# ZrrSkywalker/MonoDETR

Measured on AMD Instinct MI355X. Metric: training images/sec at B=8 per GPU, KITTI 384x1280, higher is better.
Workload: dtype bf16; 1 GPU; full MonoDETR training step (ResNet-50 + depth predictor + 3 enc / 3 dec layers, 550 train queries, 4 levels, criterion + AdamW) = BASELINE configs[2] (1 GPU) / configs[3] (DDP); global_batch=8, per_gpu_batch=8, image=3x384x1280, queries=50, precision=bf16, parallelism=dp1, grad_sync=none, prime_steps=12, launch=one hipGraph replay per iteration, cpu_affinity=NUMA node 1 of the GPU

## Files before the change

include/monodetr_amd.h:

```cpp
#ifndef MONODETR_AMD_H
#define MONODETR_AMD_H

#include <stdint.h>

#ifdef __cplusplus
extern "C" {
#endif

#define MDETR_ABI_VERSION 17

#define MDETR_F32 0
#define MDETR_F64 1
#define MDETR_BF16 2

#define MDETR_OK            0
#define MDETR_E_ARG        -1
#define MDETR_E_HIP        -2
#define MDETR_E_ALIGN      -3
#define MDETR_E_UNSUPPORTED -4

int mdetr_abi_version(void);
const char *mdetr_last_error(void);

int mdetr_msda_forward(int dtype,
                       const void *value, const int64_t *spatial_shapes, const int64_t *level_start,
                       const void *loc, const void *attn, void *out,
                       int B, int S, int M, int D, int L, int Lq, int P,
                       int device, void *stream);

int mdetr_msda_backward(int dtype,
                        const void *value, const int64_t *spatial_shapes, const int64_t *level_start,
                        const void *loc, const void *attn, const void *grad_out,
                        void *grad_value, void *grad_loc, void *grad_attn,
                        int B, int S, int M, int D, int L, int Lq, int P,
                        int device, void *stream);

int mdetr_msda_forward_cpu(int dtype,
                           const void *value, const int64_t *spatial_shapes, const int64_t *level_start,
                           const void *loc, const void *attn, void *out,
                           int B, int S, int M, int D, int L, int Lq, int P);
int mdetr_msda_backward_cpu(int dtype,
                            const void *value, const int64_t *spatial_shapes, const int64_t *level_start,
// ... 93 lines not shown
                            float alpha, float fg_weight, float bg_weight, float depth_min, float depth_max,
                            const float *grad_out, float *grad_logits, int device, void *stream);

int mdetr_adamw_step(int param_dtype, void *param, float *master, const void *grad, float *exp_avg, float *exp_avg_sq,
                     int64_t n, int64_t n_no_decay, float beta1, float beta2, float eps, float weight_decay,
                     float step_size, const float *step_size_dev, int device, void *stream);
int mdetr_adamw_step_counted(int param_dtype, void *param, float *master, const void *grad, float *exp_avg, float *exp_avg_sq,
                             int64_t n, int64_t n_no_decay, float beta1, float beta2, float eps, float weight_decay,
                             const double *step_count_dev, float lr, const double *lr_dev, int device, void *stream);
int mdetr_adamw_step_gathered(int param_dtype, void *param, float *master, const void *const *grad_ptrs, int ntensors,
                              const int *tensor_block_begin, const int64_t *flat_offsets, const int64_t *nbytes, const int *block_tensor,
                              const int64_t *block_start, int chunk_bytes, float *exp_avg, float *exp_avg_sq, int64_t n_no_decay,
                              float beta1, float beta2, float eps, float weight_decay, float step_size, const float *step_size_dev,
                              const double *step_count_dev, float lr, const double *lr_dev, int device, void *stream);

#define MDETR_TGEMM_RELU 1
#define MDETR_TGEMM_NN 2
#define MDETR_TGEMM_BIAS_F32 4
#define MDETR_TGEMM_OUT_F32 8
int mdetr_tgemm(const void *a, const void *w, const void *bias, const void *res, void *y, int64_t T, int N, int K,
                int64_t lda, int64_t ldw, int64_t ldr, int64_t ldy, int flags, float dropout_p, uint64_t seed,
                const void *seed_dev, int device, void *stream);
int mdetr_tgemm_masked(const void *a, const void *w, const void *res, const void *mask, void *y, int64_t T, int N, int K,
                       int64_t lda, int64_t ldw, int64_t ldr, int64_t ldm, int64_t ldy, int device, void *stream);
int mdetr_tgemm_f32(const void *a, const void *w, const void *bias, const void *res, void *y, int64_t T, int N, int K,
                    int64_t lda, int64_t ldw, int64_t ldr, int64_t ldy, int flags, float dropout_p, uint64_t seed,
                    const void *seed_dev, int device, void *stream);
int mdetr_tgemm_f32_masked(const void *a, const void *w, const void *res, const void *mask, void *y, int64_t T, int N, int K,
                           int64_t lda, int64_t ldw, int64_t ldr, int64_t ldm, int64_t ldy, int device, void *stream);

#define MDETR_SGEMM_NT 0
#define MDETR_SGEMM_NN 1
#define MDETR_SGEMM_TN 2
#define MDETR_SGEMM_MAX_PROBLEMS 10
#define MDETR_SGEMM_MAX_TERMS 5
typedef struct {
    const void *a, *b;
    int64_t lda, ldb;
    int32_t k, a_dtype, b_dtype, pad_;
} mdetr_sgemm_term;
typedef struct {
    mdetr_sgemm_term term[MDETR_SGEMM_MAX_TERMS];
    void *c;
    const float *bias;
    float *colsum;
    const float *mask;
    const void *res;
    int64_t ldc, ldm, ldr;
    int32_t nterm, m, n, relu_cols, c_dtype, res_dtype;
} mdetr_sgemm_problem;
int64_t mdetr_sgemm_workspace_bytes(int mode, const mdetr_sgemm_problem *problems, int nprob);
int mdetr_sgemm_grouped(int mode, const mdetr_sgemm_problem *problems, int nprob, void *workspace, int64_t workspace_bytes, int device, void *stream);

#define MDETR_KITTI_FLIP 1u
#define MDETR_KITTI_DISTORT 2u
#define MDETR_KITTI_CONTRAST_FIRST 4u
#define MDETR_KITTI_BRIGHTNESS 8u
#define MDETR_KITTI_CONTRAST 16u
#define MDETR_KITTI_SATURATION 32u
#define MDETR_KITTI_HUE 64u
typedef struct MdetrKittiImage {
    int64_t pixel_offset;
    int32_t width, height;
    uint32_t flags;
    uint32_t perm;
    float brightness, contrast, saturation, hue;
// ... 134 lines not shown
```

monodetr_amd/_capi.py:

```python
import ctypes
import os
import threading

_HERE = os.path.dirname(os.path.abspath(__file__))
LIB_PATH = os.environ.get("MDETR_LIB_PATH") or os.path.join(_HERE, "libmonodetr_amd.so")

MDETR_F32, MDETR_F64, MDETR_BF16 = 0, 1, 2
MDETR_E_UNSUPPORTED = -4
ABI_VERSION = 17

_c_int, _c_vp = ctypes.c_int, ctypes.c_void_p

SIGNATURES = {
    "mdetr_abi_version": (_c_int, []),
    "mdetr_last_error": (ctypes.c_char_p, []),
    "mdetr_msda_variant": (_c_int, [_c_int] * 5),
    "mdetr_msda_forward": (_c_int, [_c_int] + [_c_vp] * 6 + [_c_int] * 7 + [_c_int, _c_vp]),
    "mdetr_msda_backward": (_c_int, [_c_int] + [_c_vp] * 9 + [_c_int] * 7 + [_c_int, _c_vp]),
    "mdetr_msda_forward_cpu": (_c_int, [_c_int] + [_c_vp] * 6 + [_c_int] * 7),
    "mdetr_msda_backward_cpu": (_c_int, [_c_int] + [_c_vp] * 9 + [_c_int] * 7),
    "mdetr_msda_backward_ex": (_c_int, [_c_int] + [_c_vp] * 9 + [_c_int] * 7 + [_c_vp, _c_vp, _c_vp, ctypes.c_int64] + [_c_int, _c_vp]),
    "mdetr_msda_backward_workspace_bytes": (ctypes.c_int64, [_c_int, _c_vp, _c_vp] + [_c_int] * 7),
    "mdetr_msda_indices": (_c_int, [_c_int] + [_c_vp] * 3 + [_c_int] * 5 + [_c_int, _c_vp]),
    "mdetr_attn_forward": (_c_int, [_c_int] + [_c_vp] * 6 + [_c_int] * 4 + [ctypes.c_int64] * 3 + [_c_int] * 3
                           + [ctypes.c_float, ctypes.c_float, ctypes.c_uint64, _c_vp, _c_int, _c_vp]),
    "mdetr_attn_backward": (_c_int, [_c_int] + [_c_vp] * 11 + [_c_int] * 4 + [ctypes.c_int64] * 3 + [_c_int] * 3
                            + [ctypes.c_float, ctypes.c_float, ctypes.c_uint64, _c_vp, _c_int, _c_vp]),
    "mdetr_lsa_forward": (_c_int, [_c_vp] * 3 + [_c_int] * 5 + [ctypes.c_int64] * 3 + [_c_int, _c_vp]),
    "mdetr_ddn_loss_forward": (_c_int, [_c_vp] * 4 + [_c_int] * 5 + [ctypes.c_int64] * 4 + [ctypes.c_float] * 5 + [_c_vp, _c_vp, _c_int, _c_vp]),
    "mdetr_ddn_loss_backward": (_c_int, [_c_vp] * 4 + [_c_int] * 5 + [ctypes.c_int64] * 4 + [ctypes.c_float] * 5 + [_c_vp, _c_vp, _c_int, _c_vp]),
    "mdetr_pair_losses_workspace_bytes": (ctypes.c_int64, [_c_int, _c_int]),
    "mdetr_pair_losses_forward": (_c_int, [_c_vp] * 14 + [_c_int] * 6 + [ctypes.c_float, ctypes.c_float] + [_c_vp] * 4 + [_c_int, _c_vp]),
    "mdetr_pair_losses_backward": (_c_int, [_c_vp] * 13 + [_c_int] * 6 + [ctypes.c_float, ctypes.c_float] + [_c_vp] * 8 + [_c_int, _c_vp]),
    "mdetr_adamw_step": (_c_int, [_c_int] + [_c_vp] * 5 + [ctypes.c_int64] * 2 + [ctypes.c_float] * 5 + [_c_vp, _c_int, _c_vp]),
    "mdetr_adamw_step_gathered": (_c_int, [_c_int, _c_vp, _c_vp, _c_vp, _c_int] + [_c_vp] * 5 + [_c_int, _c_vp, _c_vp, ctypes.c_int64] + [ctypes.c_float] * 5
                                  + [_c_vp, _c_vp, ctypes.c_float, _c_vp, _c_int, _c_vp]),
    "mdetr_adamw_step_counted": (_c_int, [_c_int] + [_c_vp] * 5 + [ctypes.c_int64] * 2 + [ctypes.c_float] * 4 + [_c_vp, ctypes.c_float, _c_vp, _c_int, _c_vp]),
    "mdetr_tgemm": (_c_int, [_c_vp] * 5 + [ctypes.c_int64, _c_int, _c_int] + [ctypes.c_int64] * 4 + [_c_int, ctypes.c_float, ctypes.c_uint64, _c_vp, _c_int, _c_vp]),
    "mdetr_sgemm_workspace_bytes": (ctypes.c_int64, [_c_int, _c_vp, _c_int]),
    "mdetr_sgemm_grouped": (_c_int, [_c_int, _c_vp, _c_int, _c_vp, ctypes.c_int64, _c_int, _c_vp]),
    "mdetr_tgemm_masked": (_c_int, [_c_vp] * 5 + [ctypes.c_int64, _c_int, _c_int] + [ctypes.c_int64] * 5 + [_c_int, _c_vp]),
    "mdetr_tgemm_f32": (_c_int, [_c_vp] * 5 + [ctypes.c_int64, _c_int, _c_int] + [ctypes.c_int64] * 4 + [_c_int, ctypes.c_float, ctypes.c_uint64, _c_vp, _c_int, _c_vp]),
# ... 119 lines not shown
```

monodetr_amd/csrc/sgemm.hip:

```cpp
#include <hip/hip_runtime.h>
#include <stdint.h>

#include <mdetr_wave.h>

#include "msda.h"
#include "sgemm.h"

namespace mdetr {
namespace {

constexpr int kTile = 64, kSlab = 32, kPitchK = kSlab + 4, kPitchN = kTile + 4, kTnTile = 64, kTnWaves = 4, kTnMaxSplit = 16;
constexpr int kMaxTerms = 24;
constexpr int kFlagCBf16 = 1, kFlagResBf16 = 2;

struct Term {
    const void *a, *b;
    int64_t lda, ldb;
    int K, a_bf16, b_bf16, pad_;
};
struct Prob {
    void *c;
    const float *bias;
    float *colsum;
    const float *mask;
    const void *res;
    int64_t ldc, ldm, ldr;
    int M, N, relu_cols, term0, nterm, tile0, tiles_n, flags;
    int foff, pad_;
};
struct Args {
    Term t[kMaxTerms];
    Prob p[MDETR_SGEMM_MAX_PROBLEMS];
    int nprob;
    int split, flat;
    float *ws;
};

// ... 451 lines not shown
            const float *slot = red + wave * 64 * 64;
#pragma unroll
            for (int q = 0; q < 4; ++q) {
#pragma unroll
                for (int r = 0; r < 16; ++r) acc[q >> 1][q & 1][r] += slot[(q * 16 + r) * 64 + lane];
            }
        }
    }
    if (wave != 0) return;
    float sum = 0.f;
#pragma unroll
    for (int w = 0; w < kTnWaves; ++w) sum += cred[w * 64 + lane];
    const int mm = tm * kTnTile + lane;
    if (split == 1) {
#pragma unroll
        for (int q = 0; q < 4; ++q)
            epilogue_tile(P, tm * kTnTile + (q >> 1), 2, tn * kTnTile + 2 * li + (q & 1), lh, acc[q >> 1][q & 1]);
        if (P.colsum && tn == 0 && mm < PM) as_global_rw<float>(P.colsum)[mm] = sum;
        return;
    }
    MDETR_GLOBAL float *part = as_global_rw<float>(largs.ws) + static_cast<int64_t>(blockIdx.y) * largs.flat + P.foff;
#pragma unroll
    for (int q = 0; q < 4; ++q) {
        const int col = tn * kTnTile + 2 * li + (q & 1);
#pragma unroll
        for (int r = 0; r < 16; ++r) {
            const int row = tm * kTnTile + (q >> 1) + 2 * ((r & 3) + 8 * (r >> 2) + 4 * lh);
            if (row < PM && col < PN) part[static_cast<int64_t>(row) * PN + col] = acc[q >> 1][q & 1][r];
        }
    }
    if (tn == 0 && mm < PM) part[static_cast<int64_t>(PM) * PN + mm] = sum;
}

__global__ __launch_bounds__(256)
void sgemm_tn_reduce(const Args a)
{
    __shared__ __attribute__((aligned(16))) Args largs;
    {
        const unsigned *src = reinterpret_cast<const unsigned *>(&a);
        unsigned *dst = reinterpret_cast<unsigned *>(&largs);
        for (unsigned i = threadIdx.x; i < sizeof(Args) / 4; i += blockDim.x) dst[i] = src[i];
        __syncthreads();
    }
    const int f = blockIdx.x * 256 + threadIdx.x, flat = largs.flat;
    if (f >= flat) return;
    int pi = 0;
    for (int i = 1; i < largs.nprob; ++i)
        if (f >= largs.p[i].foff) pi = i;
    const Prob &P = largs.p[pi];
    const MDETR_GLOBAL float *part = as_global<float>(largs.ws) + f;
    float v = 0.f;
    for (int s2 = 0; s2 < largs.split; ++s2) v += part[static_cast<int64_t>(s2) * flat];
    const int e = f - P.foff, mn = P.M * P.N;
    if (e < mn) {
        const int row = e / P.N, col = e - row * P.N;
        const int64_t o = static_cast<int64_t>(row) * P.ldc + col;
        if (P.flags & kFlagCBf16) as_global_rw<__bf16>(P.c)[o] = static_cast<__bf16>(v);
        else as_global_rw<float>(P.c)[o] = v;
    } else if (P.colsum) {
        as_global_rw<float>(P.colsum)[e - mn] = v;
    }
}

int tn_split(const mdetr_sgemm_problem *p, int nprob)
{
    int tiles = 0, kmin = 1 << 30;
    for (int i = 0; i < nprob; ++i) {
        tiles += ((p[i].m + kTnTile - 1) / kTnTile) * ((p[i].n + kTnTile - 1) / kTnTile);
        kmin = p[i].term[0].k < kmin ? p[i].term[0].k : kmin;
    }
    int s = (768 + tiles - 1) / tiles;
    const int by_rows = kmin / (64 * kTnWaves);
    s = s < by_rows ? s : by_rows;
    return s < 1 ? 1 : (s > kTnMaxSplit ? kTnMaxSplit : s);
}

int64_t tn_flat(const mdetr_sgemm_problem *p, int nprob)
{
    int64_t f = 0;
    for (int i = 0; i < nprob; ++i) f += static_cast<int64_t>(p[i].m) * p[i].n + p[i].m;
    return f;
}

bool dtype_ok(int d) { return d == MDETR_F32 || d == MDETR_BF16; }

}

const char *sgemm_check(int mode, const mdetr_sgemm_problem *p, int nprob)
{
    if (mode != MDETR_SGEMM_NT && mode != MDETR_SGEMM_NN && mode != MDETR_SGEMM_TN) return "unknown mode";
    if (!p || nprob <= 0 || nprob > MDETR_SGEMM_MAX_PROBLEMS) return "1 .. MDETR_SGEMM_MAX_PROBLEMS problems per group";
    int terms = 0;
    for (int i = 0; i < nprob; ++i) {
        const mdetr_sgemm_problem &q = p[i];
        if (q.m <= 0 || q.n <= 0 || q.nterm <= 0 || q.nterm > MDETR_SGEMM_MAX_TERMS) return "bad shape (m, n > 0; 1 .. MDETR_SGEMM_MAX_TERMS terms)";
        if (!q.c || q.ldc < q.n || !dtype_ok(q.c_dtype)) return "bad result (null, row stride < n, or element type)";
        if (q.relu_cols < 0 || q.relu_cols > q.n) return "relu_cols outside [0, n]";
        if (q.mask && q.ldm < q.n) return "mask row stride < n";
        if (q.res && (q.ldr < q.n || !dtype_ok(q.res_dtype))) return "bad res (row stride < n, or element type)";
        if (mode == MDETR_SGEMM_TN && (q.nterm != 1 || q.bias || q.mask || q.res || q.relu_cols)) return "TN: one term, no bias / relu / mask / res";
        if (mode != MDETR_SGEMM_TN && q.colsum) return "colsum belongs to TN";
        for (int t = 0; t < q.nterm; ++t) {
            const mdetr_sgemm_term &x = q.term[t];
            if (!x.a || !x.b || x.k <= 0 || !dtype_ok(x.a_dtype) || !dtype_ok(x.b_dtype)) return "bad term (null operand, k <= 0, or element type)";
            const int64_t a_cols = mode == MDETR_SGEMM_TN ? q.m : x.k, b_cols = mode == MDETR_SGEMM_NT ? x.k : q.n;
            if (x.lda < a_cols || x.ldb < b_cols) return "operand row stride shorter than its row";
        }
        terms += q.nterm;
    }
    if (terms > kMaxTerms) return "too many terms in one group";
    if (mode == MDETR_SGEMM_TN && tn_flat(p, nprob) >= (1ll << 31)) return "TN group too large";
    return nullptr;
}

int64_t sgemm_workspace_bytes(int mode, const mdetr_sgemm_problem *p, int nprob)
{
    if (mode != MDETR_SGEMM_TN) return 0;
    const int split = tn_split(p, nprob);
    return split > 1 ? static_cast<int64_t>(split) * tn_flat(p, nprob) * 4 : 0;
}

hipError_t sgemm_launch(int mode, const mdetr_sgemm_problem *p, int nprob, void *workspace, hipStream_t st)
{
    Args a;
    a.split = 1; a.flat = 0; a.ws = nullptr;
    int tiles = 0, terms = 0;
    int64_t foff = 0;
    double flop = 0.0, bytes = 0.0;
    const int tsz = mode == MDETR_SGEMM_TN ? kTnTile : kTile;
    for (int i = 0; i < nprob; ++i) {
        const mdetr_sgemm_problem &q = p[i];
        Prob &P = a.p[i];
        P.c = q.c; P.bias = q.bias; P.colsum = q.colsum; P.mask = q.mask; P.res = q.res;
        P.ldc = q.ldc; P.ldm = q.ldm; P.ldr = q.ldr;
        P.M = q.m; P.N = q.n; P.relu_cols = q.relu_cols; P.term0 = terms; P.nterm = q.nterm;
        P.tile0 = tiles; P.tiles_n = (q.n + tsz - 1) / tsz;
        P.flags = (q.c_dtype == MDETR_BF16 ? kFlagCBf16 : 0) | (q.res && q.res_dtype == MDETR_BF16 ? kFlagResBf16 : 0);
        P.foff = static_cast<int>(foff); P.pad_ = 0;
        foff += static_cast<int64_t>(q.m) * q.n + q.m;
        tiles += ((q.m + tsz - 1) / tsz) * P.tiles_n;
        bytes += static_cast<double>(q.m) * q.n * (q.c_dtype == MDETR_BF16 ? 2.0 : 4.0) * (1.0 + (q.res ? 1.0 : 0.0)) + (q.mask ? 4.0 * q.m * q.n : 0.0);
        for (int t = 0; t < q.nterm; ++t) {
            const mdetr_sgemm_term &x = q.term[t];
            Term &T = a.t[terms++];
            T.a = x.a; T.b = x.b; T.lda = x.lda; T.ldb = x.ldb; T.K = x.k;
            T.a_bf16 = x.a_dtype == MDETR_BF16; T.b_bf16 = x.b_dtype == MDETR_BF16; T.pad_ = 0;
            flop += 2.0 * q.m * q.n * x.k;
            bytes += static_cast<double>(x.k) * (q.m * (T.a_bf16 ? 2.0 : 4.0) + q.n * (T.b_bf16 ? 2.0 : 4.0));
        }
    }
    a.nprob = nprob;
    ProfileScope prof(21, tiles, st, flop / 1e6, bytes / 1e3);
    if (mode == MDETR_SGEMM_TN) {
        a.split = tn_split(p, nprob);
        a.flat = static_cast<int>(tn_flat(p, nprob));
        a.ws = static_cast<float *>(workspace);
        hipLaunchKernelGGL(sgemm_tn_kernel, dim3(tiles, a.split), dim3(64 * kTnWaves), 0, st, a);
        if (a.split > 1) hipLaunchKernelGGL(sgemm_tn_reduce, dim3((a.flat + 255) / 256), dim3(256), 0, st, a);
    }
    else if (mode == MDETR_SGEMM_NN) hipLaunchKernelGGL(sgemm_kernel<true>, dim3(tiles), dim3(256), 0, st, a);
    else hipLaunchKernelGGL(sgemm_kernel<false>, dim3(tiles), dim3(256), 0, st, a);
    return hipGetLastError();
}

}
```

monodetr_amd/monodetr/heads.py:

```python
import os

import torch

from .. import sgemm_ext

ENABLED = os.environ.get("MDETR_HEADS") == "1"


def _heads_ok(x, bbox, dim, dep, ang, cls):
    from .depthaware_transformer import MLP
    if not ENABLED:
        return False
    if not (isinstance(bbox, MLP) and bbox.num_layers == 3 and all(isinstance(m, MLP) and m.num_layers == 2 for m in (dim, dep, ang))
            and isinstance(cls, torch.nn.Linear)):
        return False
    ps = [p for m in (bbox, dim, dep, ang, cls) for p in m.parameters()]
    if not all(p.dtype == torch.float32 and p.is_contiguous() for p in ps):
        return False
    C = x.shape[-1]
    firsts = [bbox.layers[0], dim.layers[0], dep.layers[0], ang.layers[0]]
    hid = firsts[0].out_features
    if not (all(l.in_features == C and l.out_features == hid and l.bias is not None for l in firsts) and cls.in_features == C
            and cls.bias is not None and bbox.layers[1].in_features == hid and bbox.layers[1].out_features == hid
            and all(m.layers[-1].bias is not None for m in (bbox, dim, dep, ang)) and bbox.layers[1].bias is not None):
        return False
    return x.dim() == 3 and x.is_contiguous() and sgemm_ext.usable(x.view(-1, C), *ps) and not torch.is_autocast_enabled()


class _HeadsLevel(torch.autograd.Function):

    @staticmethod
    def forward(ctx, x, w1b, b1b, w2b, b2b, w3b, b3b, w1d, b1d, wd, bd, w1p, b1p, wp, bp, w1a, b1a, wa, ba, wc, bc):
        ctx.set_materialize_grads(False)
        B, Q, C = x.shape
        T, hid = B * Q, w1b.shape[0]
        x2 = x.view(T, C)
        new = lambda n: torch.empty((T, n), dtype=torch.float32, device=x.device)
        h1, h2 = new(4 * hid), new(hid)
        delta, size, depth, angle, logits = new(w3b.shape[0]), new(wd.shape[0]), new(wp.shape[0]), new(wa.shape[0]), new(wc.shape[0])
        P, G = sgemm_ext.Problem, sgemm_ext.grouped
        sl = [slice(i * hid, (i + 1) * hid) for i in range(4)]
        G(sgemm_ext.NT, [P([(x2, w)], h1[:, s], bias=b, relu_cols=True) for w, b, s in zip((w1b, w1d, w1p, w1a), (b1b, b1d, b1p, b1a), sl)]
          + [P([(x2, wc)], logits, bias=bc)])
        G(sgemm_ext.NT, [P([(h1[:, sl[0]], w2b)], h2, bias=b2b, relu_cols=True), P([(h1[:, sl[1]], wd)], size, bias=bd),
                         P([(h1[:, sl[2]], wp)], depth, bias=bp), P([(h1[:, sl[3]], wa)], angle, bias=ba)])
        G(sgemm_ext.NT, [P([(h2, w3b)], delta, bias=b3b)])
        ctx.save_for_backward(x, h1, h2, w1b, w2b, w3b, w1d, wd, w1p, wp, w1a, wa, wc)
        shape = lambda t: t.view(B, Q, -1)
        return shape(delta), shape(size), shape(depth), shape(angle), shape(logits), x.view_as(x)

    @staticmethod
    @torch.autograd.function.once_differentiable
    def backward(ctx, g_delta, g_size, g_depth, g_angle, g_logits, g_skip):
        x, h1, h2, w1b, w2b, w3b, w1d, wd, w1p, wp, w1a, wa, wc = ctx.saved_tensors
        B, Q, C = x.shape
        T, hid = B * Q, w1b.shape[0]
        x2 = x.view(T, C)

        def flat(g, n):
            if g is None:
                return torch.zeros((T, n), dtype=torch.float32, device=x.device)
            return g.reshape(T, n).to(torch.float32).contiguous()
        g_delta, g_size, g_depth, g_angle, g_logits = (flat(g, w.shape[0]) for g, w in
                                                       ((g_delta, w3b), (g_size, wd), (g_depth, wp), (g_angle, wa), (g_logits, wc)))
        P, G = sgemm_ext.Problem, sgemm_ext.grouped
        sl = [slice(i * hid, (i + 1) * hid) for i in range(4)]
        new = lambda *s: torch.empty(s, dtype=torch.float32, device=x.device)
        dh2, dh1 = new(T, hid), new(T, 4 * hid)
        G(sgemm_ext.NN, [P([(g_delta, w3b)], dh2, mask=h2)])
        G(sgemm_ext.NN, [P([(g, w)], dh1[:, s], mask=h1[:, s]) for g, w, s in zip((dh2, g_size, g_depth, g_angle), (w2b, wd, wp, wa), sl)])
        dx = None
        if ctx.needs_input_grad[0]:
            dx = torch.empty_like(x)
            skip = g_skip.reshape(T, C) if g_skip is not None else None
            if skip is not None and not (skip.stride(1) == 1 and skip.dtype in (torch.float32, torch.bfloat16)):
                skip = skip.contiguous()
            G(sgemm_ext.NN, [P([(dh1[:, s], w) for s, w in zip(sl, (w1b, w1d, w1p, w1a))] + [(g_logits, wc)], dx.view(T, C), res=skip)])
        outs = {}
        jobs = []
        for key, dy, act, w in (("3b", g_delta, h2, w3b), ("2b", dh2, h1[:, sl[0]], w2b), ("d", g_size, h1[:, sl[1]], wd),
                                ("p", g_depth, h1[:, sl[2]], wp), ("a", g_angle, h1[:, sl[3]], wa),
                                ("1b", dh1[:, sl[0]], x2, w1b), ("1d", dh1[:, sl[1]], x2, w1d), ("1p", dh1[:, sl[2]], x2, w1p),
                                ("1a", dh1[:, sl[3]], x2, w1a), ("c", g_logits, x2, wc)):
            dw, db = torch.empty_like(w), new(w.shape[0])
            outs[key] = (dw, db)
            jobs.append(P([(dy, act)], dw, colsum=db))
        G(sgemm_ext.TN, jobs)
        o = outs
        return (dx, o["1b"][0], o["1b"][1], o["2b"][0], o["2b"][1], o["3b"][0], o["3b"][1], o["1d"][0], o["1d"][1], o["d"][0], o["d"][1],
                o["1p"][0], o["1p"][1], o["p"][0], o["p"][1], o["1a"][0], o["1a"][1], o["a"][0], o["a"][1], o["c"][0], o["c"][1])


def heads_level(x, bbox, dim, dep, ang, cls):
    if not _heads_ok(x, bbox, dim, dep, ang, cls):
        return None
    lb, ld, lp, la = bbox.layers, dim.layers, dep.layers, ang.layers
    return _HeadsLevel.apply(x, lb[0].weight, lb[0].bias, lb[1].weight, lb[1].bias, lb[2].weight, lb[2].bias,
                             ld[0].weight, ld[0].bias, ld[1].weight, ld[1].bias, lp[0].weight, lp[0].bias, lp[1].weight, lp[1].bias,
                             la[0].weight, la[0].bias, la[1].weight, la[1].bias, cls.weight, cls.bias)
```

monodetr_amd/sgemm_ext.py:

```python
import ctypes

import torch

from . import _capi

_backend = None
NT, NN, TN = 0, 1, 2
MAX_PROBLEMS, MAX_TERMS = 10, 5


class _Term(ctypes.Structure):
    _fields_ = [("a", ctypes.c_void_p), ("b", ctypes.c_void_p), ("lda", ctypes.c_int64), ("ldb", ctypes.c_int64),
                ("k", ctypes.c_int32), ("a_dtype", ctypes.c_int32), ("b_dtype", ctypes.c_int32), ("pad_", ctypes.c_int32)]


class _Problem(ctypes.Structure):
    _fields_ = [("term", _Term * MAX_TERMS), ("c", ctypes.c_void_p), ("bias", ctypes.c_void_p), ("colsum", ctypes.c_void_p),
                ("mask", ctypes.c_void_p), ("res", ctypes.c_void_p), ("ldc", ctypes.c_int64), ("ldm", ctypes.c_int64),
                ("ldr", ctypes.c_int64), ("nterm", ctypes.c_int32), ("m", ctypes.c_int32), ("n", ctypes.c_int32),
                ("relu_cols", ctypes.c_int32), ("c_dtype", ctypes.c_int32), ("res_dtype", ctypes.c_int32)]


def _lib():
    return _backend if _backend is not None else _capi.lib()


def _code(t):
    if t.dtype == torch.float32:
        return _capi.MDETR_F32
    if t.dtype == torch.bfloat16:
        return _capi.MDETR_BF16
    raise TypeError("sgemm: fp32 or bf16 operands, got %s" % t.dtype)


def _mat(t, what):
    if not (t.dim() == 2 and t.stride(1) == 1 and t.stride(0) >= t.shape[1]):
        raise ValueError("sgemm: %s must be 2-D with unit column stride, got shape %s strides %s" % (what, tuple(t.shape), t.stride()))
    return t


def usable(*tensors):
    for t in tensors:
        if t is None:
            continue
        if not ((t.is_cuda or _backend is not None) and t.dtype in (torch.float32, torch.bfloat16) and t.dim() in (1, 2) and t.stride(-1) == 1):
            return False
    return True


class Problem:

    def __init__(self, terms, out, bias=None, relu_cols=0, mask=None, res=None, colsum=None):
        self.terms, self.out, self.bias, self.mask, self.res, self.colsum = list(terms), out, bias, mask, res, colsum
        self.relu_cols = out.shape[1] if relu_cols is True else int(relu_cols)


def grouped(mode, problems):
    if not 0 < len(problems) <= MAX_PROBLEMS:
        raise ValueError("sgemm: 1 .. %d problems per group" % MAX_PROBLEMS)
    arr = (_Problem * len(problems))()
    dev = problems[0].out.device
    for q, pr in zip(arr, problems):
        out = _mat(pr.out, "out")
        M, N = out.shape
        if len(pr.terms) > MAX_TERMS:
            raise ValueError("sgemm: at most %d terms per problem" % MAX_TERMS)
        for i, (A, B) in enumerate(pr.terms):
            A, B = _mat(A, "A"), _mat(B, "B")
            if mode == NT:
                K = A.shape[1]
                ok = A.shape == (M, K) and B.shape == (N, K)
            elif mode == NN:
                K = A.shape[1]
                ok = A.shape == (M, K) and B.shape == (K, N)
            else:
                K = A.shape[0]
                ok = A.shape == (K, M) and B.shape == (K, N)
            if not ok:
                raise ValueError("sgemm: term %d shapes A %s B %s do not give [%d, %d] in mode %d" % (i, tuple(A.shape), tuple(B.shape), M, N, mode))
            t = q.term[i]
            t.a, t.b, t.lda, t.ldb, t.k, t.a_dtype, t.b_dtype = A.data_ptr(), B.data_ptr(), A.stride(0), B.stride(0), K, _code(A), _code(B)
        q.nterm, q.m, q.n, q.relu_cols = len(pr.terms), M, N, pr.relu_cols
        q.c, q.ldc, q.c_dtype = out.data_ptr(), out.stride(0), _code(out)
        if pr.bias is not None:
            assert pr.bias.dtype == torch.float32 and pr.bias.shape == (N,) and pr.bias.is_contiguous()
            q.bias = pr.bias.data_ptr()
        if pr.mask is not None:
            mk = _mat(pr.mask, "mask")
            assert mk.dtype == torch.float32 and mk.shape == (M, N)
            q.mask, q.ldm = mk.data_ptr(), mk.stride(0)
        if pr.res is not None:
            rs = _mat(pr.res, "res")
            assert rs.shape == (M, N)
            q.res, q.ldr, q.res_dtype = rs.data_ptr(), rs.stride(0), _code(rs)
        if pr.colsum is not None:
            assert pr.colsum.dtype == torch.float32 and pr.colsum.shape == (M,) and pr.colsum.is_contiguous()
            q.colsum = pr.colsum.data_ptr()
    parr = ctypes.cast(arr, ctypes.c_void_p)
    need = _lib().mdetr_sgemm_workspace_bytes(mode, parr, len(problems)) if mode == TN else 0
    ws = torch.empty(need, dtype=torch.uint8, device=dev) if need > 0 else None
    rc = -1 if need < 0 else _lib().mdetr_sgemm_grouped(mode, parr, len(problems), ws.data_ptr() if ws is not None else None, max(need, 0),
                                                        dev.index if dev.type == "cuda" else -1,
                                                        torch.cuda.current_stream(dev).cuda_stream if dev.type == "cuda" else None)
    if rc != 0:
        msg = _lib().mdetr_last_error()
        raise RuntimeError("mdetr_sgemm_grouped failed (code %d): %s" % (rc, msg.decode() if msg else "?"))
```

Measured before the change: 501.6 images/sec.

## Add bf16-split MFMA grouped GEMM kernel for prediction heads

Adds a new grouped GEMM kernel that splits fp32 operands into up to three bf16 planes and accumulates the cross products with bf16 MFMA. It uses a three-deep register prefetch pipeline, transposed LDS fragment reads, and optional 32-row tiles with a k-half reduction. The heads' forward, backward and weight-gradient GEMMs opt into it when activations are bf16. The aim is to replace the older GEMM path with a matrix-core path and better occupancy. In exchange it runs extra MFMA products for fp32 operands and adds a large amount of template code.

```diff
diff --git a/include/monodetr_amd.h b/include/monodetr_amd.h
--- a/include/monodetr_amd.h
+++ b/include/monodetr_amd.h
@@ -7,7 +7,7 @@
 extern "C" {
 #endif
 
-#define MDETR_ABI_VERSION 17
+#define MDETR_ABI_VERSION 18
 
 #define MDETR_F32 0
 #define MDETR_F64 1
@@ -167,6 +167,7 @@
 #define MDETR_SGEMM_NT 0
 #define MDETR_SGEMM_NN 1
 #define MDETR_SGEMM_TN 2
+#define MDETR_SGEMM_SPLIT 16
 #define MDETR_SGEMM_MAX_PROBLEMS 10
 #define MDETR_SGEMM_MAX_TERMS 5
 typedef struct {
diff --git a/monodetr_amd/_capi.py b/monodetr_amd/_capi.py
--- a/monodetr_amd/_capi.py
+++ b/monodetr_amd/_capi.py
@@ -7,7 +7,7 @@
 
 MDETR_F32, MDETR_F64, MDETR_BF16 = 0, 1, 2
 MDETR_E_UNSUPPORTED = -4
-ABI_VERSION = 17
+ABI_VERSION = 18
 
 _c_int, _c_vp = ctypes.c_int, ctypes.c_void_p
 
diff --git a/monodetr_amd/csrc/sgemm.hip b/monodetr_amd/csrc/sgemm.hip
--- a/monodetr_amd/csrc/sgemm.hip
+++ b/monodetr_amd/csrc/sgemm.hip
@@ -3,6 +3,8 @@
 
 #include <mdetr_wave.h>
 
+#include "mdetr_split.h"
+#include "mdetr_tune.h"
 #include "msda.h"
 #include "sgemm.h"
 
@@ -520,6 +522,258 @@
     if (tn == 0 && mm < PM) part[static_cast<int64_t>(PM) * PN + mm] = sum;
 }
 
+constexpr int kPitchC = kSlab + 8, kPitchR = kTile + 32;
+constexpr int kPlaneR = kSlab * kPitchR;
+constexpr int plane_c(int rows) { return rows * kPitchC; }
+static_assert((kPitchC * 2) % 16 == 0 && (kPitchR * 2) % 8 == 0 && (plane_c(32) * 2) % 16 == 0 && (kPlaneR * 2) % 16 == 0, "aligned fragment reads");
+
+__device__ __forceinline__ bf16x8 tr_fragment(const __bf16 *rows, int pitch, int lane)
+{
+    const int s = lane & 15, grp = lane >> 4;
+    const __bf16 *p = rows + (8 * (grp >> 1) + (s >> 2)) * pitch + 16 * (grp & 1) + 4 * (s & 3);
+    const bf16x4 lo = lds_read_tr4(p), hi = lds_read_tr4(p + 4 * pitch);
+    bf16x8 f;
+#pragma unroll
+    for (int i = 0; i < 4; ++i) { f[i] = lo[i]; f[4 + i] = hi[i]; }
+    return f;
+}
+
+struct SplitOp {
+    const void *base;
+    int64_t ld;
+    int lim, t0;
+    bool vec;
+};
+
+template <bool KR, bool FULL> __device__ __forceinline__ int op_valid(const SplitOp &o, int r, int q, int p, int k0, int k_end)
+{
+    if (FULL) return 4;
+    if (KR) return k0 + r + 16 * p < k_end ? clamp04(o.lim - (o.t0 + q)) : 0;
+    return o.t0 + r + 32 * p < o.lim ? clamp04(k_end - (k0 + q)) : 0;
+}
+template <bool KR, bool FULL> __device__ __forceinline__ int64_t op_off(const SplitOp &o, int r, int q, int p, int k0)
+{
+    if (KR) return static_cast<int64_t>(k0 + r + 16 * p) * o.ld + o.t0 + q;
+    return static_cast<int64_t>(FULL ? min(o.t0 + r + 32 * p, o.lim - 1) : o.t0 + r + 32 * p) * o.ld + k0 + q;
+}
+
+template <bool BF> __device__ __forceinline__ void put_planes(__bf16 *plane0, int plane, int dst, const f32x4 &v)
+{
+    const float x[4] = {v.x, v.y, v.z, v.w};
+    bf16x4 h, m, l;
+    if (BF) {
+#pragma unroll
+        for (int i = 0; i < 4; ++i) h[i] = static_cast<__bf16>(x[i]);
+        *reinterpret_cast<bf16x4 *>(plane0 + dst) = h;
+    } else {
+        split4(x, h, m, l);
+        *reinterpret_cast<bf16x4 *>(plane0 + dst) = h;
+        *reinterpret_cast<bf16x4 *>(plane0 + plane + dst) = m;
+        *reinterpret_cast<bf16x4 *>(plane0 + 2 * plane + dst) = l;
+    }
+}
+
+template <int MODE, int TM> struct SplitGeo {
+    static constexpr bool AKR = MODE == MDETR_SGEMM_TN, BKR = MODE != MDETR_SGEMM_NT;
+    static constexpr int PA = AKR ? kPlaneR : plane_c(TM), PB = BKR ? kPlaneR : plane_c(kTile);
+    static constexpr int NPA = AKR ? 2 : TM / 32;
+    static constexpr int KS = TM == 64 ? 2 : 1;
+    static_assert(TM == 64 || (TM == 32 && !AKR), "32-row tiles: NT / NN");
+};
+
+template <typename G, bool ABF, bool BBF>
+__device__ __forceinline__ void split_products(const __bf16 *Ab, const __bf16 *Bb, int wm, int wn, int kh, int lane, f32x16 &acc, f32x16 &accb,
+                                               bool want_cs)
+{
+    constexpr int NA = ABF ? 1 : 3, NB = BBF ? 1 : 3;
+    constexpr int term_a[6] = {2, 0, 1, 1, 0, 0}, term_b[6] = {0, 2, 1, 0, 1, 0};
+    const int li = lane & 31, lh = lane >> 5;
+    bf16x8 ones;
+#pragma unroll
+    for (int i = 0; i < 8; ++i) ones[i] = static_cast<__bf16>(1.0f);
+#pragma unroll
+    for (int j = 0; j < G::KS; ++j) {
+        const int ks = G::KS == 2 ? j : kh;
+        bf16x8 af[NA], bf[NB];
+#pragma unroll
+        for (int p = 0; p < NA; ++p) {
+            if (G::AKR) af[p] = tr_fragment(Ab + p * G::PA + ks * 16 * kPitchR + wm * 32, kPitchR, lane);
+            else af[p] = *reinterpret_cast<const bf16x8 *>(Ab + p * G::PA + (wm * 32 + li) * kPitchC + 16 * ks + 8 * lh);
+        }
+#pragma unroll
+        for (int p = 0; p < NB; ++p) {
+            if (G::BKR) bf[p] = tr_fragment(Bb + p * G::PB + ks * 16 * kPitchR + wn * 32, kPitchR, lane);
+            else bf[p] = *reinterpret_cast<const bf16x8 *>(Bb + p * G::PB + (wn * 32 + li) * kPitchC + 16 * ks + 8 * lh);
+        }
+#pragma unroll
+        for (int t = 0; t < 6; ++t)
+            if (term_a[t] < NA && term_b[t] < NB) acc = mfma_bf16(af[term_a[t] < NA ? term_a[t] : 0], bf[term_b[t] < NB ? term_b[t] : 0], acc);
+        if (want_cs) {
+#pragma unroll
+            for (int p = NA - 1; p >= 0; --p) accb = mfma_bf16(af[p], ones, accb);
+        }
+    }
+}
+
+struct SplitCtx {
+    SplitOp A, B;
+    int ar, aq, br, bq;
+    int wm, wn, kh, lane;
+    bool want_cs;
+};
+
+template <typename G, bool ABF, bool BBF, bool AFULL, bool BFULL>
+__device__ __forceinline__ void split_term(const SplitCtx &c, int k_begin, int k_end, __bf16 *Ap, __bf16 *Bp, f32x16 &acc, f32x16 &accb)
+{
+    constexpr bool AKR = G::AKR, BKR = G::BKR;
+    const int slabs = (k_end - k_begin + kSlab - 1) / kSlab;
+    if (slabs <= 0) return;
+    u32x4 ra[3][2], rb[3][2];
+    auto load = [&](int s, u32x4 (&xa)[2], u32x4 (&xb)[2]) {
+        const int k0 = k_begin + min(s, slabs - 1) * kSlab;
+#pragma unroll
+        for (int p = 0; p < 2; ++p) {
+            if (p < G::NPA) xa[p] = raw4(c.A.base, ABF, op_off<AKR, AFULL>(c.A, c.ar, c.aq, p, k0), op_valid<AKR, AFULL>(c.A, c.ar, c.aq, p, k0, k_end), AFULL);
+            xb[p] = raw4(c.B.base, BBF, op_off<BKR, BFULL>(c.B, c.br, c.bq, p, k0), op_valid<BKR, BFULL>(c.B, c.br, c.bq, p, k0, k_end), BFULL);
+        }
+    };
+    auto store = [&](int s, const u32x4 (&xa)[2], const u32x4 (&xb)[2]) {
+        const int k0 = k_begin + s * kSlab;
+#pragma unroll
+        for (int p = 0; p < 2; ++p) {
+            const int da = AKR ? (c.ar + 16 * p) * kPitchR + c.aq : (c.ar + 32 * p) * kPitchC + c.aq;
+            const int db = BKR ? (c.br + 16 * p) * kPitchR + c.bq : (c.br + 32 * p) * kPitchC + c.bq;
+            if (p < G::NPA) put_planes<ABF>(Ap, G::PA, da, decode4(xa[p], ABF, op_valid<AKR, AFULL>(c.A, c.ar, c.aq, p, k0, k_end), AFULL));
+            put_planes<BBF>(Bp, G::PB, db, decode4(xb[p], BBF, op_valid<BKR, BFULL>(c.B, c.br, c.bq, p, k0, k_end), BFULL));
+        }
+    };
+    if (!AFULL && !BFULL && slabs <= 2) {
+        for (int s2 = 0; s2 < slabs; ++s2) {
+            load(s2, ra[0], rb[0]);
+            store(s2, ra[0], rb[0]);
+            __syncthreads();
+            split_products<G, ABF, BBF>(Ap, Bp, c.wm, c.wn, c.kh, c.lane, acc, accb, c.want_cs);
+            __syncthreads();
+        }
+        return;
+    }
+    load(0, ra[0], rb[0]);
+    load(1, ra[1], rb[1]);
+    load(2, ra[2], rb[2]);
+    store(0, ra[0], rb[0]);
+    __syncthreads();
+#define MDETR_SGEMM_SPLIT_STEP(FREE, NEXT)                                                                             \
+    {                                                                                                                  \
+        load(s2 + 3, ra[FREE], rb[FREE]);                                                                              \
+        split_products<G, ABF, BBF>(Ap, Bp, c.wm, c.wn, c.kh, c.lane, acc, accb, c.want_cs);                           \
+        __syncthreads();                                                                                               \
+        if (s2 + 1 < slabs) store(s2 + 1, ra[NEXT], rb[NEXT]);                                                         \
+        __syncthreads();                                                                                               \
+        if (++s2 >= slabs) break;                                                                                      \
+    }
+    for (int s2 = 0;;) {
+        MDETR_SGEMM_SPLIT_STEP(0, 1)
+        MDETR_SGEMM_SPLIT_STEP(1, 2)
+        MDETR_SGEMM_SPLIT_STEP(2, 0)
+    }
+#undef MDETR_SGEMM_SPLIT_STEP
+}
+
+template <typename G>
+__device__ __forceinline__ void split_term_dispatch(const SplitCtx &c, int abf, int bbf, int k_begin, int k_end, __bf16 *Ap, __bf16 *Bp,
+                                                    f32x16 &acc, f32x16 &accb)
+{
+    const int k_mid = k_begin + (k_end - k_begin) / kSlab * kSlab;
+    const bool afull = c.A.vec && (!G::AKR || c.A.t0 + kTile <= c.A.lim), bfull = c.B.vec && (!G::BKR || c.B.t0 + kTile <= c.B.lim);
+#pragma unroll 1
+    for (int pass = 0; pass < 2; ++pass) {
+        const int kb = pass == 0 ? k_begin : k_mid, ke = pass == 0 ? k_mid : k_end;
+        if (ke <= kb) continue;
+        const int v = (abf ? 8 : 0) | (bbf ? 4 : 0) | (pass == 0 && afull ? 2 : 0) | (pass == 0 && bfull ? 1 : 0);
+#define MDETR_SGEMM_SPLIT_CASE(V)                                                                                                              \
+        case V: split_term<G, ((V) & 8) != 0, ((V) & 4) != 0, ((V) & 2) != 0, ((V) & 1) != 0>(c, kb, ke, Ap, Bp, acc, accb); break;
+        switch (v) {
+            MDETR_SGEMM_SPLIT_CASE(0) MDETR_SGEMM_SPLIT_CASE(1) MDETR_SGEMM_SPLIT_CASE(2) MDETR_SGEMM_SPLIT_CASE(3)
+            MDETR_SGEMM_SPLIT_CASE(4) MDETR_SGEMM_SPLIT_CASE(5) MDETR_SGEMM_SPLIT_CASE(6) MDETR_SGEMM_SPLIT_CASE(7)
+            MDETR_SGEMM_SPLIT_CASE(8) MDETR_SGEMM_SPLIT_CASE(9) MDETR_SGEMM_SPLIT_CASE(10) MDETR_SGEMM_SPLIT_CASE(11)
+            MDETR_SGEMM_SPLIT_CASE(12) MDETR_SGEMM_SPLIT_CASE(13) MDETR_SGEMM_SPLIT_CASE(14) MDETR_SGEMM_SPLIT_CASE(15)
+        }
+#undef MDETR_SGEMM_SPLIT_CASE
+    }
+}
+
+template <int MODE, int TM>
+__global__ __launch_bounds__(256, 3)
+void sgemm_split_kernel(const Args a)
+{
+    typedef SplitGeo<MODE, TM> G;
+    constexpr bool AKR = G::AKR, BKR = G::BKR;
+    __shared__ __attribute__((aligned(16))) __bf16 Ap[3 * G::PA];
+    __shared__ __attribute__((aligned(16))) __bf16 Bp[3 * G::PB];
+    __shared__ __attribute__((aligned(16))) Args largs;
+    static_assert(sizeof(Bp) >= 2 * 16 * 64 * sizeof(float), "the k-halves of a 32-row tile meet in the B planes");
+    const int tile = blockIdx.x;
+    const Prob &P = stage_args(a, &largs, tile);
+    const Term *terms = &largs.t[wave_uniform(P.term0)];
+    const int tiles_n = wave_uniform(P.tiles_n), lt = tile - wave_uniform(P.tile0);
+    const int PM = wave_uniform(P.M), PN = wave_uniform(P.N), tm = lt / tiles_n, tn = lt - tm * tiles_n;
+    const int tid = threadIdx.x, lane = tid & 63, wave = tid >> 6, li = lane & 31, lh = lane >> 5;
+    SplitCtx c;
+    c.ar = AKR ? tid >> 4 : tid >> 3; c.aq = AKR ? (tid & 15) << 2 : (tid & 7) << 2;
+    c.br = BKR ? tid >> 4 : tid >> 3; c.bq = BKR ? (tid & 15) << 2 : (tid & 7) << 2;
+    c.wm = TM == 64 ? wave >> 1 : 0; c.kh = TM == 64 ? 0 : wave >> 1; c.wn = wave & 1; c.lane = lane;
+    c.want_cs = MODE == MDETR_SGEMM_TN && tn == 0 && c.wn == 0;
+    c.A.lim = PM; c.A.t0 = tm * TM; c.B.lim = PN; c.B.t0 = tn * kTile;
+
+    f32x16 acc, accb;
+#pragma unroll
+    for (int r = 0; r < 16; ++r) acc[r] = accb[r] = 0.f;
+
+    const int nterm = MODE == MDETR_SGEMM_TN ? 1 : wave_uniform(P.nterm), split = wave_uniform(largs.split);
+    for (int t = 0; t < nterm; ++t) {
+        const Term T = uniform_term(terms[t]);
+        c.A.base = T.a; c.A.ld = T.lda; c.A.vec = vec_ok(T.a, T.lda, T.a_bf16);
+        c.B.base = T.b; c.B.ld = T.ldb; c.B.vec = vec_ok(T.b, T.ldb, T.b_bf16);
+        int k_begin = 0, k_end = T.K;
+        if (MODE == MDETR_SGEMM_TN) {
+            const int chunk = ((T.K + split * kSlab - 1) / (split * kSlab)) * kSlab;
+            k_begin = min(T.K, static_cast<int>(blockIdx.y) * chunk);
+            k_end = min(T.K, k_begin + chunk);
+        }
+        split_term_dispatch<G>(c, T.a_bf16, T.b_bf16, k_begin, k_end, Ap, Bp, acc, accb);
+    }
+    if (TM == 32) {
+        float *red = reinterpret_cast<float *>(&Bp[0]) + c.wn * 16 * 64;
+        if (c.kh == 1) {
+#pragma unroll
+            for (int r = 0; r < 16; ++r) red[r * 64 + lane] = acc[r];
+        }
+        __syncthreads();
+        if (c.kh == 1) return;
+#pragma unroll
+        for (int r = 0; r < 16; ++r) acc[r] += red[r * 64 + lane];
+    }
+    const int row0 = tm * TM + c.wm * 32, col = tn * kTile + c.wn * 32 + li;
+    if (MODE != MDETR_SGEMM_TN || split == 1) {
+        epilogue_tile(P, row0, 1, col, lh, acc);
+        if (MODE == MDETR_SGEMM_TN && P.colsum && c.want_cs && li == 0) {
+#pragma unroll
+            for (int r = 0; r < 16; ++r) {
+                const int row = row0 + (r & 3) + 8 * (r >> 2) + 4 * lh;
+                if (row < PM) as_global_rw<float>(P.colsum)[row] = accb[r];
+            }
+        }
+        return;
+    }
+    MDETR_GLOBAL float *part = as_global_rw<float>(largs.ws) + static_cast<int64_t>(blockIdx.y) * largs.flat + P.foff;
+#pragma unroll
+    for (int r = 0; r < 16; ++r) {
+        const int row = row0 + (r & 3) + 8 * (r >> 2) + 4 * lh;
+        if (row < PM && col < PN) part[static_cast<int64_t>(row) * PN + col] = acc[r];
+        if (c.want_cs && li == 0 && row < PM) part[static_cast<int64_t>(PM) * PN + row] = accb[r];
+    }
+}
+
 __global__ __launch_bounds__(256)
 void sgemm_tn_reduce(const Args a)
 {
@@ -550,19 +804,44 @@
     }
 }
 
-int tn_split(const mdetr_sgemm_problem *p, int nprob)
+int tn_split(const mdetr_sgemm_problem *p, int nprob, int target = 768)
 {
     int tiles = 0, kmin = 1 << 30;
     for (int i = 0; i < nprob; ++i) {
         tiles += ((p[i].m + kTnTile - 1) / kTnTile) * ((p[i].n + kTnTile - 1) / kTnTile);
         kmin = p[i].term[0].k < kmin ? p[i].term[0].k : kmin;
     }
-    int s = (768 + tiles - 1) / tiles;
+    int s = (target + tiles - 1) / tiles;
     const int by_rows = kmin / (64 * kTnWaves);
     s = s < by_rows ? s : by_rows;
     return s < 1 ? 1 : (s > kTnMaxSplit ? kTnMaxSplit : s);
 }
 
+constexpr int kSplitPlaces = 768;
+int tn_split_form(const mdetr_sgemm_problem *p, int nprob)
+{
+    int tiles = 0, kmin = 1 << 30;
+    for (int i = 0; i < nprob; ++i) {
+        tiles += ((p[i].m + kTile - 1) / kTile) * ((p[i].n + kTile - 1) / kTile);
+        kmin = p[i].term[0].k < kmin ? p[i].term[0].k : kmin;
+    }
+    int places = tune_int("sgemm_split_tn_wgs", 0);
+    if (places < 1 || places > 16384) places = kSplitPlaces;
+    int s = places / tiles;
+    const int by_rows = kmin / 128;
+    s = s < by_rows ? s : by_rows;
+    return s < 1 ? 1 : (s > kTnMaxSplit ? kTnMaxSplit : s);
+}
+
+int split_tile_rows(const mdetr_sgemm_problem *p, int nprob)
+{
+    const int forced = tune_int("sgemm_split_tm", 0);
+    if (forced == 32 || forced == 64) return forced;
+    int tiles = 0;
+    for (int i = 0; i < nprob; ++i) tiles += ((p[i].m + kTile - 1) / kTile) * ((p[i].n + kTile - 1) / kTile);
+    return tiles <= kSplitPlaces / 2 ? 32 : 64;
+}
+
 int64_t tn_flat(const mdetr_sgemm_problem *p, int nprob)
 {
     int64_t f = 0;
@@ -572,10 +851,17 @@
 
 bool dtype_ok(int d) { return d == MDETR_F32 || d == MDETR_BF16; }
 
+bool want_split(int mode)
+{
+    const int forced = tune_int("sgemm_split", -1);
+    return forced == 0 ? false : (forced == 1 ? true : (mode & MDETR_SGEMM_SPLIT) != 0);
+}
+
 }
 
 const char *sgemm_check(int mode, const mdetr_sgemm_problem *p, int nprob)
 {
+    mode &= ~MDETR_SGEMM_SPLIT;
     if (mode != MDETR_SGEMM_NT && mode != MDETR_SGEMM_NN && mode != MDETR_SGEMM_TN) return "unknown mode";
     if (!p || nprob <= 0 || nprob > MDETR_SGEMM_MAX_PROBLEMS) return "1 .. MDETR_SGEMM_MAX_PROBLEMS problems per group";
     int terms = 0;
@@ -603,19 +889,24 @@
 
 int64_t sgemm_workspace_bytes(int mode, const mdetr_sgemm_problem *p, int nprob)
 {
+    const bool split_form = want_split(mode);
+    mode &= ~MDETR_SGEMM_SPLIT;
     if (mode != MDETR_SGEMM_TN) return 0;
-    const int split = tn_split(p, nprob);
+    const int split = split_form ? tn_split_form(p, nprob) : tn_split(p, nprob);
     return split > 1 ? static_cast<int64_t>(split) * tn_flat(p, nprob) * 4 : 0;
 }
 
 hipError_t sgemm_launch(int mode, const mdetr_sgemm_problem *p, int nprob, void *workspace, hipStream_t st)
 {
+    const bool split_form = want_split(mode);
+    mode &= ~MDETR_SGEMM_SPLIT;
     Args a;
     a.split = 1; a.flat = 0; a.ws = nullptr;
     int tiles = 0, terms = 0;
     int64_t foff = 0;
     double flop = 0.0, bytes = 0.0;
     const int tsz = mode == MDETR_SGEMM_TN ? kTnTile : kTile;
+    const int tsz_m = split_form && mode != MDETR_SGEMM_TN ? split_tile_rows(p, nprob) : tsz;
     for (int i = 0; i < nprob; ++i) {
         const mdetr_sgemm_problem &q = p[i];
         Prob &P = a.p[i];
@@ -626,7 +917,7 @@
         P.flags = (q.c_dtype == MDETR_BF16 ? kFlagCBf16 : 0) | (q.res && q.res_dtype == MDETR_BF16 ? kFlagResBf16 : 0);
         P.foff = static_cast<int>(foff); P.pad_ = 0;
         foff += static_cast<int64_t>(q.m) * q.n + q.m;
-        tiles += ((q.m + tsz - 1) / tsz) * P.tiles_n;
+        tiles += ((q.m + tsz_m - 1) / tsz_m) * P.tiles_n;
         bytes += static_cast<double>(q.m) * q.n * (q.c_dtype == MDETR_BF16 ? 2.0 : 4.0) * (1.0 + (q.res ? 1.0 : 0.0)) + (q.mask ? 4.0 * q.m * q.n : 0.0);
         for (int t = 0; t < q.nterm; ++t) {
             const mdetr_sgemm_term &x = q.term[t];
@@ -639,13 +930,20 @@
     }
     a.nprob = nprob;
     ProfileScope prof(21, tiles, st, flop / 1e6, bytes / 1e3);
+#define MDETR_SGEMM_SPLIT_LAUNCH(MODE, TM, GRID) hipLaunchKernelGGL((sgemm_split_kernel<MODE, TM>), GRID, dim3(256), 0, st, a);
     if (mode == MDETR_SGEMM_TN) {
-        a.split = tn_split(p, nprob);
+        a.split = split_form ? tn_split_form(p, nprob) : tn_split(p, nprob);
         a.flat = static_cast<int>(tn_flat(p, nprob));
         a.ws = static_cast<float *>(workspace);
-        hipLaunchKernelGGL(sgemm_tn_kernel, dim3(tiles, a.split), dim3(64 * kTnWaves), 0, st, a);
+        if (split_form) MDETR_SGEMM_SPLIT_LAUNCH(MDETR_SGEMM_TN, 64, dim3(tiles, a.split))
+        else hipLaunchKernelGGL(sgemm_tn_kernel, dim3(tiles, a.split), dim3(64 * kTnWaves), 0, st, a);
         if (a.split > 1) hipLaunchKernelGGL(sgemm_tn_reduce, dim3((a.flat + 255) / 256), dim3(256), 0, st, a);
     }
+    else if (split_form && mode == MDETR_SGEMM_NN && tsz_m == 32) MDETR_SGEMM_SPLIT_LAUNCH(MDETR_SGEMM_NN, 32, dim3(tiles))
+    else if (split_form && mode == MDETR_SGEMM_NN) MDETR_SGEMM_SPLIT_LAUNCH(MDETR_SGEMM_NN, 64, dim3(tiles))
+    else if (split_form && tsz_m == 32) MDETR_SGEMM_SPLIT_LAUNCH(MDETR_SGEMM_NT, 32, dim3(tiles))
+    else if (split_form) MDETR_SGEMM_SPLIT_LAUNCH(MDETR_SGEMM_NT, 64, dim3(tiles))
+#undef MDETR_SGEMM_SPLIT_LAUNCH
     else if (mode == MDETR_SGEMM_NN) hipLaunchKernelGGL(sgemm_kernel<true>, dim3(tiles), dim3(256), 0, st, a);
     else hipLaunchKernelGGL(sgemm_kernel<false>, dim3(tiles), dim3(256), 0, st, a);
     return hipGetLastError();
diff --git a/monodetr_amd/monodetr/heads.py b/monodetr_amd/monodetr/heads.py
--- a/monodetr_amd/monodetr/heads.py
+++ b/monodetr_amd/monodetr/heads.py
@@ -5,6 +5,10 @@
 from .. import sgemm_ext
 
 ENABLED = os.environ.get("MDETR_HEADS") == "1"
+
+
+def _split_form(x):
+    return x.dtype == torch.bfloat16
 
 
 def _heads_ok(x, bbox, dim, dep, ang, cls):
@@ -41,10 +45,10 @@
         P, G = sgemm_ext.Problem, sgemm_ext.grouped
         sl = [slice(i * hid, (i + 1) * hid) for i in range(4)]
         G(sgemm_ext.NT, [P([(x2, w)], h1[:, s], bias=b, relu_cols=True) for w, b, s in zip((w1b, w1d, w1p, w1a), (b1b, b1d, b1p, b1a), sl)]
-          + [P([(x2, wc)], logits, bias=bc)])
+          + [P([(x2, wc)], logits, bias=bc)], split=_split_form(x))
         G(sgemm_ext.NT, [P([(h1[:, sl[0]], w2b)], h2, bias=b2b, relu_cols=True), P([(h1[:, sl[1]], wd)], size, bias=bd),
-                         P([(h1[:, sl[2]], wp)], depth, bias=bp), P([(h1[:, sl[3]], wa)], angle, bias=ba)])
-        G(sgemm_ext.NT, [P([(h2, w3b)], delta, bias=b3b)])
+                         P([(h1[:, sl[2]], wp)], depth, bias=bp), P([(h1[:, sl[3]], wa)], angle, bias=ba)], split=_split_form(x))
+        G(sgemm_ext.NT, [P([(h2, w3b)], delta, bias=b3b)], split=_split_form(x))
         ctx.save_for_backward(x, h1, h2, w1b, w2b, w3b, w1d, wd, w1p, wp, w1a, wa, wc)
         shape = lambda t: t.view(B, Q, -1)
         return shape(delta), shape(size), shape(depth), shape(angle), shape(logits), x.view_as(x)
@@ -67,15 +71,17 @@
         sl = [slice(i * hid, (i + 1) * hid) for i in range(4)]
         new = lambda *s: torch.empty(s, dtype=torch.float32, device=x.device)
         dh2, dh1 = new(T, hid), new(T, 4 * hid)
-        G(sgemm_ext.NN, [P([(g_delta, w3b)], dh2, mask=h2)])
-        G(sgemm_ext.NN, [P([(g, w)], dh1[:, s], mask=h1[:, s]) for g, w, s in zip((dh2, g_size, g_depth, g_angle), (w2b, wd, wp, wa), sl)])
+        G(sgemm_ext.NN, [P([(g_delta, w3b)], dh2, mask=h2)], split=_split_form(x))
+        G(sgemm_ext.NN, [P([(g, w)], dh1[:, s], mask=h1[:, s]) for g, w, s in zip((dh2, g_size, g_depth, g_angle), (w2b, wd, wp, wa), sl)],
+          split=_split_form(x))
         dx = None
         if ctx.needs_input_grad[0]:
             dx = torch.empty_like(x)
             skip = g_skip.reshape(T, C) if g_skip is not None else None
             if skip is not None and not (skip.stride(1) == 1 and skip.dtype in (torch.float32, torch.bfloat16)):
                 skip = skip.contiguous()
-            G(sgemm_ext.NN, [P([(dh1[:, s], w) for s, w in zip(sl, (w1b, w1d, w1p, w1a))] + [(g_logits, wc)], dx.view(T, C), res=skip)])
+            G(sgemm_ext.NN, [P([(dh1[:, s], w) for s, w in zip(sl, (w1b, w1d, w1p, w1a))] + [(g_logits, wc)], dx.view(T, C), res=skip)],
+              split=_split_form(x))
         outs = {}
         jobs = []
         for key, dy, act, w in (("3b", g_delta, h2, w3b), ("2b", dh2, h1[:, sl[0]], w2b), ("d", g_size, h1[:, sl[1]], wd),
@@ -85,7 +91,7 @@
             dw, db = torch.empty_like(w), new(w.shape[0])
             outs[key] = (dw, db)
             jobs.append(P([(dy, act)], dw, colsum=db))
-        G(sgemm_ext.TN, jobs)
+        G(sgemm_ext.TN, jobs, split=_split_form(x))
         o = outs
         return (dx, o["1b"][0], o["1b"][1], o["2b"][0], o["2b"][1], o["3b"][0], o["3b"][1], o["1d"][0], o["1d"][1], o["d"][0], o["d"][1],
                 o["1p"][0], o["1p"][1], o["p"][0], o["p"][1], o["1a"][0], o["1a"][1], o["a"][0], o["a"][1], o["c"][0], o["c"][1])
diff --git a/monodetr_amd/sgemm_ext.py b/monodetr_amd/sgemm_ext.py
--- a/monodetr_amd/sgemm_ext.py
+++ b/monodetr_amd/sgemm_ext.py
@@ -6,6 +6,7 @@
 
 _backend = None
 NT, NN, TN = 0, 1, 2
+SPLIT = 16
 MAX_PROBLEMS, MAX_TERMS = 10, 5
 
 
@@ -55,7 +56,7 @@
         self.relu_cols = out.shape[1] if relu_cols is True else int(relu_cols)
 
 
-def grouped(mode, problems):
+def grouped(mode, problems, split=False):
     if not 0 < len(problems) <= MAX_PROBLEMS:
         raise ValueError("sgemm: 1 .. %d problems per group" % MAX_PROBLEMS)
     arr = (_Problem * len(problems))()
@@ -97,7 +98,8 @@
             assert pr.colsum.dtype == torch.float32 and pr.colsum.shape == (M,) and pr.colsum.is_contiguous()
             q.colsum = pr.colsum.data_ptr()
     parr = ctypes.cast(arr, ctypes.c_void_p)
-    need = _lib().mdetr_sgemm_workspace_bytes(mode, parr, len(problems)) if mode == TN else 0
+    base, mode = mode, (mode | SPLIT if split else mode)
+    need = _lib().mdetr_sgemm_workspace_bytes(mode, parr, len(problems)) if base == TN else 0
     ws = torch.empty(need, dtype=torch.uint8, device=dev) if need > 0 else None
     rc = -1 if need < 0 else _lib().mdetr_sgemm_grouped(mode, parr, len(problems), ws.data_ptr() if ws is not None else None, max(need, 0),
                                                         dev.index if dev.type == "cuda" else -1,
```

New measurement: 506.6 images/sec, median of 6. 1.01x the previous value.
